# A-SHOJAEI/adverse-weather-semantic-segmentation-robustness-benchmark

Measured on AMD Instinct MI355X. Metric: images/sec (1024x2048, 5 weather conds, ensemble eval), higher is better.
Workload: dtype f32 (results float32; attention, gemm_1x1, winograd_3x3, segformer_head on 3xf16 split operands: 22-bit operands, f32 accumulate)

## Files before the change

adverse_weather_semantic_segmentation_robustness_benchmark_amd/_native.py:

```python
from __future__ import annotations

import ctypes as C
from pathlib import Path

import numpy as np
import torch

_PKG = Path(__file__).resolve().parent
LIB_PATH = _PKG / "libawseg_hip.so"

U8, I64 = 0, 1
COMBINE_WEIGHTED, COMBINE_MAXCONF, COMBINE_MEAN = 0, 1, 2
LOSS_CE, LOSS_FOCAL = 0, 1
ACT_NONE, ACT_RELU, ACT_GELU = 0, 1, 2
MAX_CLASSES = 32

c_i, c_i64, c_u64, c_f, c_d, c_p = C.c_int, C.c_int64, C.c_uint64, C.c_float, C.c_double, C.c_void_p

FOG_JOB = np.dtype([("image", "<i4"), ("_pad", "<i4"), ("beta", "<f8"), ("atmos", "<f8"), ("seed", "<u8")], align=True)
NIGHT_JOB = np.dtype([("image", "<i4"), ("_pad", "<i4"), ("brightness", "<f8"), ("intensity", "<f8"), ("seed", "<u8")], align=True)
PRIM_JOB = np.dtype([("image", "<i4"), ("prim_offset", "<i4"), ("prim_count", "<i4"), ("blur_ksize", "<i4"), ("intensity", "<f8")], align=True)
WEATHER_JOB = np.dtype([("kind", "<i4"), ("image", "<i4"), ("a", "<f8"), ("b", "<f8"), ("seed", "<u8"), ("prim_offset", "<i4"), ("prim_count", "<i4")], align=True)
WEATHER_CLEAN, WEATHER_FOG, WEATHER_RAIN, WEATHER_SNOW, WEATHER_NIGHT = 0, 1, 2, 3, 4
assert FOG_JOB.itemsize == 32 and NIGHT_JOB.itemsize == 32 and PRIM_JOB.itemsize == 24 and WEATHER_JOB.itemsize == 40

SIGNATURES = {
    "awseg_abi_version": (c_i, []),
    "awseg_header_hash": (C.c_uint64, []),
    "awseg_error_string": (C.c_char_p, [c_i]),
    "awseg_device_count": (c_i, []),
    "awseg_metrics_workspace": (c_i64, [c_i64, c_i, c_i64]),
    "awseg_confusion_accumulate": (c_i, [c_p, c_i, c_p, c_i, c_i64, c_i, c_i, c_i, c_p, c_p, c_p, c_p]),
    "awseg_argmax": (c_i, [c_p, c_i64, c_i, c_i64, c_p, c_i, c_p]),
    "awseg_combine_argmax_confusion": (c_i, [c_p, c_p, c_i64, c_i, c_i64, c_i, c_p, c_p, c_p, c_p, c_i, c_p, c_i, c_i,
                                            c_i, c_p, c_p, c_i, c_p, c_p, c_p]),
    "awseg_argmax_confusion": (c_i, [c_p, c_i64, c_i, c_i64, c_p, c_i, c_p, c_i, c_i, c_i, c_p, c_p, c_i, c_p, c_p, c_p]),
    "awseg_normalize": (c_i, [c_p, c_i64, c_i, c_i, c_p, c_i, c_p, c_p, c_p, c_p]),
    "awseg_synthetic_depth": (c_i, [c_i, c_i, c_p, c_i, c_p, c_p, c_p, c_p]),
    "awseg_conv3x3_winograd_nhwc": (c_i, [c_p, c_i, c_i, c_i, c_i, c_i, c_i, c_p, c_p, c_p, c_i, c_p, c_p, c_p, c_p]),
    "awseg_gemm_bias_act": (c_i, [c_p, c_p, c_p, c_p, c_i, c_p, c_i64, c_i, c_i, c_p, C.c_size_t, c_p]),
    "awseg_gemm_tune": (c_i, [c_p, c_p, c_p, c_i, c_i, c_p, c_i64, c_i, c_i, c_p, C.c_size_t, c_p]),
    "awseg_gemm_split_weights": (c_i, [c_p, c_i, c_i, c_p, c_p]),
    "awseg_gemm_split_weight_halfs": (c_i64, [c_i, c_i]),
    "awseg_gemm_split_bias_act": (c_i, [c_p, c_p, c_p, c_p, c_i, c_p, c_i64, c_i, c_i, c_p]),
    "awseg_gemm_bf16_weights": (c_i, [c_p, c_i, c_i, c_p, c_p]),
    "awseg_gemm_bf16_weight_halfs": (c_i64, [c_i, c_i]),
    "awseg_gemm_bf16_bias_act": (c_i, [c_p, c_p, c_p, c_p, c_i, c_p, c_i64, c_i, c_i, c_p]),
    "awseg_conv3x3_winograd_bf16_nhwc": (c_i, [c_p, c_i, c_i, c_i, c_i, c_i, c_i, c_p, c_p, c_p, c_i, c_p, c_p, c_p, c_p]),
    "awseg_attention_d32_bf16": (c_i, [c_p, c_p, c_p, c_p, c_i, c_i, c_i, c_i, c_f, c_p]),
    "awseg_attention_d32_split_workspace": (c_i64, [c_i, c_i, c_i]),
    "awseg_attention_d32_split_ws": (c_i, [c_p, c_p, c_p, c_i, c_p, c_i, c_i, c_i, c_i, c_f, c_p, c_p]),
    "awseg_attention_d32_packed_kv": (c_i, [c_p, c_p, c_p, c_i, c_i, c_i, c_i, c_f, c_i, c_p]),
    "awseg_dwconv3x3_upcat_nhwc": (c_i, [c_p, c_i, c_i, c_i, c_p, c_i, c_i64, c_i, c_i, c_p, c_p, c_p]),
    "awseg_winograd_split_weight_halfs": (c_i64, [c_i, c_i]),
    "awseg_conv3x3_winograd_split_nhwc": (c_i, [c_p, c_i, c_i, c_i, c_i, c_i, c_i, c_p, c_p, c_p, c_i, c_p, c_p, c_p, c_p]),
    "awseg_upconv_forms_floats": (c_i64, [c_i, c_i, c_i]),
    "awseg_upconv_forms": (c_i, [c_p, c_i, c_i, c_i, c_i, c_p, c_p, c_p]),
    "awseg_depth_head_fused": (c_i, [c_p, c_i, c_i, c_i, c_i, c_p, c_i, c_p, c_p, c_p, c_p, c_p]),
    "awseg_im2col_nhwc": (c_i, [c_p, c_i64, c_i, c_i, c_i, c_i, c_i, c_i, c_i, c_i, c_i, c_p, c_p]),
    "awseg_attention_d32": (c_i, [c_p, c_p, c_p, c_p, c_i, c_i, c_i, c_i, c_f, c_p]),
    "awseg_attention_d32_split": (c_i, [c_p, c_p, c_p, c_p, c_i, c_i, c_i, c_i, c_f, c_p]),
    "awseg_depth_upsample_combine": (c_i, [c_p, c_p, c_i, c_i, c_i, c_i, c_i, c_p, c_p, c_p, c_p]),
    "awseg_lut3_apply": (c_i, [c_p, c_i, c_i, c_i, c_p, c_i, c_p, c_p, c_p]),
    "awseg_local_contrast": (c_i, [c_p, c_i, c_i, c_i, c_p, c_p]),
    "awseg_depth_estimate_workspace": (C.c_size_t, [c_i]),
    "awseg_depth_estimate": (c_i, [c_p, c_i, c_i, c_i, c_p, c_p, c_p, c_p, c_p]),
    "awseg_fog_apply": (c_i, [c_p, c_i, c_i, c_p, c_i, c_p, c_p, c_p, c_p, c_p, c_p]),
    "awseg_fog_fused": (c_i, [c_p, c_i, c_i, c_p, c_i, c_p, c_p, c_p, c_p, c_p, c_p, c_p, c_p]),
    "awseg_night_apply": (c_i, [c_p, c_i, c_i, c_p, c_i, c_p, c_p, c_p, c_p, c_p, c_p, c_p]),
    "awseg_rain_apply": (c_i, [c_p, c_i, c_i, c_p, c_i, c_p, c_p, c_p, c_p, c_p, c_p, c_p]),
    "awseg_snow_apply": (c_i, [c_p, c_i, c_i, c_p, c_i, c_p, c_p, c_p, c_p, c_p, c_p, c_p]),
    "awseg_weather_batch": (c_i, [c_p, c_i, c_i, c_p, c_i, c_p, c_p, c_p, c_p, c_p, c_p, c_p, c_p, c_p, c_p]),
    "awseg_streak_workspace": (c_i64, [c_i, c_i, c_i]),
    "awseg_fog_density_field": (c_i, [c_p, c_i, c_i64, c_u64, c_p, c_p, c_p]),
    "awseg_loss_partials": (c_i64, [c_i64, c_i64]),
    "awseg_fog_ce_forward": (c_i, [c_p, c_p, c_i, c_p, c_i64, c_i, c_i64, c_i, c_f, c_p, c_p, c_p, c_p, c_p]),
    "awseg_fog_ce_backward": (c_i, [c_p, c_p, c_i, c_p, c_i64, c_i, c_i64, c_i, c_f, c_p, c_p, c_p]),
    "awseg_density_workspace": (c_i64, [c_i64, c_i64]),
    "awseg_fog_density_from_depth": (c_i, [c_p, c_i64, c_i, c_i, c_p, c_p, c_p]),
    "awseg_segformer_head_fused": (c_i, [c_p, c_i64, c_i, c_i, c_i, c_i, c_i, c_p, c_p, c_p, c_p, c_i, c_p, c_p]),
    "awseg_segformer_head_fused_split": (c_i, [c_p, c_i64, c_i, c_i, c_i, c_i, c_i, c_p, c_p, c_p, c_p, c_i, c_p, c_p]),
    "awseg_upconv3x3_bn_relu": (c_i, [c_p, c_i64, c_i, c_i, c_i, c_i, c_i, c_p, c_p, c_p, c_i, c_p]),
    "awseg_upconv3x3_linear": (c_i, [c_p, c_i64, c_i, c_i, c_i, c_i, c_i, c_p, c_p, c_i, c_p]),
    "awseg_upconv3x3_adjoint": (c_i, [c_p, c_i64, c_i, c_i, c_i, c_i, c_i, c_p, c_p]),
    "awseg_aspp_depthwise3": (c_i, [c_p, c_i64, c_i, c_i, c_i, c_p, c_i, c_i, c_i, c_p, c_p]),
    "awseg_aspp_depthwise3_mean": (c_i, [c_p, c_i64, c_i, c_i, c_i, c_p, c_i, c_i, c_i, c_p, c_p, c_p]),
# ... 148 lines not shown
```

adverse_weather_semantic_segmentation_robustness_benchmark_amd/csrc/build.py:

```python
from __future__ import annotations

import os
import shutil
import subprocess
import sys
from concurrent.futures import ThreadPoolExecutor
from pathlib import Path

CSRC = Path(__file__).resolve().parent
PKG = CSRC.parent
LIB = PKG / "libawseg_hip.so"
SOURCES = ["core.hip", "metrics.hip", "weather.hip", "loss.hip", "heads.hip", "backbone.hip", "depth.hip", "wino.hip", "gemm.hip", "attn.hip", "gemm_split.hip", "gemm_split3.hip", "wino_split.hip", "depthfuse.hip", "mixffn.hip", "dwtrain.hip", "bntrain.hip", "smallops.hip", "calib.hip", "consistency.hip", "deptheval.hip", "failure.hip"]
ARCH = "gfx950"
HEADER = PKG.parent / "include" / "awseg.h"


def header_hash() -> int:
    import hashlib
    return int(hashlib.sha256(HEADER.read_bytes()).hexdigest()[:15], 16)


EXTRA_FLAGS = {"attn.hip": ["-DAWSEG_ATTN_SPLIT_WAVES=" + os.environ.get("AWSEG_ATTN_SPLIT_WAVES", "2")], "wino.hip": ["-fno-slp-vectorize"], "wino_split.hip": ["-fno-slp-vectorize", "-DAWSEG_WS_ASM_PK"],
               "core.hip": ["-DAWSEG_HEADER_HASH=0x%xULL" % header_hash()]}


def hipcc() -> str:
    for cand in (os.environ.get("HIPCC"), "/opt/rocm/bin/hipcc", shutil.which("hipcc")):
        if cand and Path(cand).exists():
            return cand
    raise RuntimeError("hipcc not found (need ROCm's hipcc to build libawseg_hip.so)")


def _flags():
    return [f"--offload-arch={ARCH}", "-O3", "-std=c++17", "-fPIC", "-ffp-contract=off",
            "-fvisibility=hidden", "-Wall", "-Wno-unused-function", "-Wno-inline-asm"]


STAMP = PKG / "libawseg_hip.flags"


def _flag_stamp() -> str:
    return repr((_flags(), sorted(EXTRA_FLAGS.items()), SOURCES))


def needs_build() -> bool:
# ... 38 lines not shown
```

adverse_weather_semantic_segmentation_robustness_benchmark_amd/models/deeplab.py:

```python
from __future__ import annotations

import os

from typing import List

import torch
import torch.nn as nn
import torch.nn.functional as F

from .. import ops


class Conv2d(nn.Conv2d):

    linear_in_training = True
    keep_channels_last = os.environ.get("AWSEG_TRAIN_KEEP_CL", "1") != "0"
    matmul_nchw = os.environ.get("AWSEG_TRAIN_MATMUL_NCHW", "1") != "0"

    def forward(self, x: torch.Tensor) -> torch.Tensor:
        if (Conv2d.linear_in_training and x.is_cuda and torch.is_grad_enabled() and self.kernel_size == (1, 1) and self.groups == 1
                and self.padding == (0, 0) and x.dim() == 4 and x.shape[2] * x.shape[3] > 1):
            if self.stride != (1, 1):
                x = x[:, :, ::self.stride[0], ::self.stride[1]]
            b, c, h, w = x.shape
# ... 208 lines not shown
            dw, gmean = ops.aspp_depthwise3_mean(xl, wdw, aspp.rates)
        else:
            dw, gmean = ops.aspp_depthwise3(xl, wdw, aspp.rates), None
        dw = dw.view(3, B * h * w, Cin)
        if gmean is None:
            gmean = xl.mean(dim=(1, 2))
        pool = aspp.convs[4]
        pw_, pbn_ = pool[1].weight.view(Cout, Cin), pool[2]
        if xl.is_cuda and xl.dtype == torch.float32:
            def fold_pool():
                s_, b_ = _bn_fold(pbn_)
                return (pw_ * s_[:, None]).contiguous(), b_.contiguous()
            w1f, b1f = fused.cached(pbn_, "aspp_pool_fold", (pw_, pbn_.weight, pbn_.bias, pbn_.running_mean, pbn_.running_var), fold_pool)
            g2 = ops.aspp_pool_branch(gmean, w1f, b1f, parts[4], pb)
        else:
            g2 = branch(gmean, pw_, pbn_) @ parts[4].t() + pb
        acc = g2[:, None, :].expand(B, h * w, Cout).contiguous().view(B * h * w, Cout)
        ys = [branch(flat, aspp.convs[0][0].weight.view(Cout, Cin), aspp.convs[0][1])]
        for r in range(3):
            mod = aspp.convs[1 + r]
            ys.append(branch(dw[r], mod[0][1].weight.view(Cout, Cin), mod[1]))
        done = None
        if ops.ASPP_PIECES and ops.GEMM_SPLIT and ops.PRECISION != "bf16" and acc.is_cuda and Cout % 32 == 0:
            wcat = fused.cached(aspp.project[0], "proj_pieces", (parts[0], parts[1], parts[2], parts[3]),
                                lambda: ops.gemm_split_weights(torch.cat(parts[:4], dim=1).contiguous()))
            done = ops.gemm_split_pieces(ys, wcat, zero_bias, 1, residual=acc, out=acc)
        if done is None:
            for i, y in enumerate(ys):
                ops.gemm_bias_act(y, parts[i], zero_bias, 1 if i == 3 else 0, residual=acc, out=acc, w_split=psplit[i])
        out = acc
        return out.view(B, h, w, Cout).permute(0, 3, 1, 2)

    @torch.no_grad()
    def forward_fused(self, *features):
        from . import fused
        from .. import _native as N
        a = self.aspp_fused(features[-1])
        a = fused.separable_bn_relu(a, self.aspp[1], self.aspp[2])
        hi = fused.conv_bn_act(features[-4], self.block1[0], self.block1[1], N.ACT_RELU)
        dwc, pwc = self.block2[0][0], self.block2[0][1]
        d = ops.dwconv3x3_upcat(fused.nhwc_view(a), fused.nhwc_view(hi), fused.dw_taps(dwc))
        B, H4, W4, Cc = d.shape
        w, shift = fused.folded_conv_bn(pwc, self.block2[1])
        w2 = w.view(w.shape[0], Cc)
        y = ops.gemm_bias_act(d.view(B * H4 * W4, Cc), w2, shift, N.ACT_RELU, w_split=fused.split_weights(pwc, w2, B * H4 * W4))
        return y.view(B, H4, W4, -1).permute(0, 3, 1, 2)


class SegmentationHead(nn.Sequential):
    def __init__(self, in_ch, out_ch, kernel_size=1, upsampling=4):
        super().__init__(Conv2d(in_ch, out_ch, kernel_size, padding=kernel_size // 2),
                         nn.UpsamplingBilinear2d(scale_factor=upsampling) if upsampling > 1 else nn.Identity(),
                         nn.Identity())


class DeepLabV3Plus(nn.Module):

    def __init__(self, encoder_name="resnet50", classes=19, encoder_output_stride=16, decoder_channels=256,
                 decoder_atrous_rates=(12, 24, 36), upsampling=4):
        super().__init__()
        self.encoder = ResNetEncoder(encoder_name, encoder_output_stride)
        self.decoder = DeepLabV3PlusDecoder(self.encoder.out_channels, decoder_channels, decoder_atrous_rates,
                                            encoder_output_stride)
        self.segmentation_head = SegmentationHead(decoder_channels, classes, 1, upsampling)
        for m in list(self.decoder.modules()) + list(self.segmentation_head.modules()):
            if isinstance(m, nn.Conv2d):
                nn.init.kaiming_uniform_(m.weight, mode="fan_in", nonlinearity="relu")
                if m.bias is not None:
                    nn.init.constant_(m.bias, 0)
            elif isinstance(m, nn.BatchNorm2d):
                nn.init.constant_(m.weight, 1)
                nn.init.constant_(m.bias, 0)
        nn.init.xavier_uniform_(self.segmentation_head[0].weight)

    def forward(self, x):
        feats = self.encoder(x)
        return self.segmentation_head(self.decoder(*feats))

    @torch.no_grad()
    def forward_fused(self, x, return_features=False):
        from . import fused
        feats = fused.resnet_features(self.encoder, x)
        dec = self.decoder.forward_fused(*feats)
        head = self.segmentation_head[0]
        if head.kernel_size == (1, 1):
            dl = fused.nhwc_view(dec)
            Bq, H4, W4, Cd = dl.shape
            y2 = ops.gemm_bias_act(dl.reshape(Bq * H4 * W4, Cd), head.weight.view(head.out_channels, Cd), head.bias, 0,
                                   w_split=fused.split_weights(head, head.weight.view(head.out_channels, Cd), Bq * H4 * W4))
            low = y2.view(Bq, H4, W4, -1).permute(0, 3, 1, 2)
        else:
            low = head(dec).contiguous()
        up = self.segmentation_head[1]
        if isinstance(up, nn.UpsamplingBilinear2d) and low.is_cuda and low.dtype == torch.float32:
            f = int(up.scale_factor)
            out = ops.upsample_bilinear(low, (low.shape[2] * f, low.shape[3] * f), True)
        else:
            out = up(low)
        return (out, feats[-1]) if return_features else out
```

adverse_weather_semantic_segmentation_robustness_benchmark_amd/ops.py:

```python
from __future__ import annotations

import math
import os

import ctypes as C
from typing import Optional, Sequence

import numpy as np
import torch

from . import _native as N

IMAGENET_MEAN = np.array([0.485, 0.456, 0.406], dtype=np.float32)
IMAGENET_STD = np.array([0.229, 0.224, 0.225], dtype=np.float32)
NIGHT_GAINS = np.array([0.8, 0.85, 1.2], dtype=np.float32)
CONDITIONS = ("clean", "fog", "rain", "snow", "night")


def gaussian_taps(sigma: float = 2.0, truncate: float = 4.0) -> np.ndarray:
    radius = int(truncate * float(sigma) + 0.5)
    x = np.arange(-radius, radius + 1)
    phi = np.exp(-0.5 / (sigma * sigma) * x ** 2)
    return phi / phi.sum()

# ... 1058 lines not shown
    if k != kh * kw * c:
        raise N.AwsegError(f"conv_gemm_split: weights have K = {k}, the convolution needs {kh * kw * c}")
    if not _split_weights_intact(w_split, n, k):
        raise N.AwsegError("w_split lost its 16-byte trailer (weight exponent): pass the tensor gemm_split_weights returned, not a copy")
    ho = (h + 2 * pad - dilation * (kh - 1) - 1) // stride + 1
    wo = (w + 2 * pad - dilation * (kw - 1) - 1) // stride + 1
    out = torch.empty(b, ho, wo, n, dtype=torch.float32, device=x.device)
    N.call("awseg_conv_gemm_split_bias_act", N.ptr(x), b, h, w, c, kh, kw, stride, pad, dilation, N.ptr(w_split), N.ptr(bias),
           N.ptr(residual), act, N.ptr(out), n, N.stream())
    return out


def im2col_nhwc(x: torch.Tensor, kh: int, kw: int, stride: int, pad: int, dilation: int = 1, k_padded: Optional[int] = None):
    x = x.contiguous()
    b, h, w, c = x.shape
    k = kh * kw * c
    kp = k if k_padded is None else int(k_padded)
    ho = (h + 2 * pad - dilation * (kh - 1) - 1) // stride + 1
    wo = (w + 2 * pad - dilation * (kw - 1) - 1) // stride + 1
    cols = torch.empty(b * ho * wo, kp, dtype=torch.float32, device=x.device)
    N.call("awseg_im2col_nhwc", N.ptr(x), b, h, w, c, kh, kw, stride, pad, dilation, kp, N.ptr(cols), N.stream())
    return cols, ho, wo


def dwconv3x3_upcat(a: torch.Tensor, hi: torch.Tensor, w9: torch.Tensor) -> torch.Tensor:
    a, hi = a.contiguous(), hi.contiguous()
    b, h, w, ca = a.shape
    _, H, W, ch = hi.shape
    out = torch.empty(b, H, W, ca + ch, dtype=torch.float32, device=a.device)
    N.call("awseg_dwconv3x3_upcat_nhwc", N.ptr(a), h, w, ca, N.ptr(hi), ch, b, H, W, N.ptr(w9.contiguous()), N.ptr(out), N.stream())
    return out


ATTENTION_SPLIT = os.environ.get("AWSEG_ATTN_SPLIT", "1") != "0"


def attention_d32(q: torch.Tensor, k: torch.Tensor, v: torch.Tensor, heads: int, scale: float,
                  split: Optional[bool] = None) -> torch.Tensor:
    q, k, v = q.contiguous(), k.contiguous(), v.contiguous()
    b, nq, c = q.shape
    out = torch.empty_like(q)
    if split is None and PRECISION == "bf16":
        sym = "awseg_attention_d32_bf16"
    else:
        sym = "awseg_attention_d32_split" if (ATTENTION_SPLIT if split is None else split) else "awseg_attention_d32"
    if sym == "awseg_attention_d32_split" and _wants_kv_image(nq, k.shape[1]):
        _attention_split_ws(q, k, v, 0, out, b, heads, nq, k.shape[1], scale)
        return out
    N.call(sym, N.ptr(q), N.ptr(k), N.ptr(v), N.ptr(out), b, heads, nq, k.shape[1], float(scale), N.stream())
    return out


ATTN_KV_IMAGE = os.environ.get("AWSEG_ATTN_KV_IMAGE", "1") != "0"


def _wants_kv_image(nq: int, nkv: int) -> bool:
    return ATTN_KV_IMAGE and nq >= 8 * nkv


def _attention_split_ws(q, k, v, pitch, out, b, heads, nq, nkv, scale):
    nbytes = int(N.lib().awseg_attention_d32_split_workspace(b, heads, nkv))
    ws = N.workspace.get(q.device, nbytes, tag="attn%d" % torch.cuda.current_stream(q.device).cuda_stream)
    N.call("awseg_attention_d32_split_ws", N.ptr(q), N.ptr_strided(k), N.ptr_strided(v), int(pitch), N.ptr(out), b, heads, nq, nkv, float(scale),
           N.ptr(ws), N.stream())


# ... 153 lines not shown
```

include/awseg.h:

```cpp
#ifndef AWSEG_H
#define AWSEG_H

#include <stddef.h>
#include <stdint.h>

#ifdef __cplusplus
extern "C" {
#endif

typedef void* awseg_stream_t;

#define AWSEG_EINVAL   (-1)
#define AWSEG_ERANGE   (-2)
#define AWSEG_EALIGN   (-3)

#define AWSEG_U8   0
#define AWSEG_I64  1

#define AWSEG_COMBINE_WEIGHTED  0
#define AWSEG_COMBINE_MAXCONF   1
#define AWSEG_COMBINE_MEAN      2

#define AWSEG_LOSS_CE     0
#define AWSEG_LOSS_FOCAL  1
// ... 160 lines not shown
                            float* out, int channels_last, awseg_stream_t stream);

int awseg_aspp_depthwise3(const float* x, int64_t batch, int h, int w, int channels,
                          const float* wdw, int rate0, int rate1, int rate2,
                          float* out, awseg_stream_t stream);
int awseg_aspp_depthwise3_mean(const float* x, int64_t batch, int h, int w, int channels, const float* wdw,
                               int rate0, int rate1, int rate2, float* out, float* mean_out, awseg_stream_t stream);

#define AWSEG_ACT_NONE 0
#define AWSEG_ACT_RELU 1
#define AWSEG_ACT_GELU 2
int awseg_dwconv3x3_nhwc(const float* x, int64_t batch, int height, int width, int channels, int dilation,
                         const float* w9, const float* bias, int act, float* out, awseg_stream_t stream);

int awseg_conv3x3_winograd_nhwc(const float* x, int batch, int height, int width, int cin, int cout, int dilation,
                                const float* u, const float* shift, const float* residual, int act,
                                const float* w2, const float* b2, float* out, awseg_stream_t stream);

int awseg_gemm_bias_act(const float* x, const float* w, const float* bias, const float* residual, int act,
                        float* out, int64_t m, int n, int k, void* workspace, size_t workspace_bytes,
                        awseg_stream_t stream);

int awseg_gemm_tune(const float* x, const float* w, const float* bias, int has_residual, int act,
                    float* scratch_out, int64_t m, int n, int k, void* workspace, size_t workspace_bytes,
                    awseg_stream_t stream);

int64_t awseg_gemm_split_weight_halfs(int n, int k);
int awseg_gemm_split_weights(const float* w, int n, int k, uint16_t* w_split, awseg_stream_t stream);
int awseg_gemm_split_bias_act(const float* x, const uint16_t* w_split, const float* bias, const float* residual, int act,
                              float* out, int64_t m, int n, int k, awseg_stream_t stream);

int awseg_dwconv3x3_upcat_nhwc(const float* a, int a_height, int a_width, int a_channels, const float* hi, int hi_channels,
                               int64_t batch, int height, int width, const float* w9, float* out, awseg_stream_t stream);

int64_t awseg_winograd_split_weight_halfs(int cin, int cout);

int64_t awseg_upconv_forms_floats(int h, int w, int cmid);
int awseg_upconv_forms(const float* g9, int batch, int cmid, int h, int w, const float* shift, float* forms, awseg_stream_t stream);
int awseg_depth_head_fused(const float* forms, int batch, int h, int w, int cmid, const uint16_t* u_split, int u_is_bf16,
                           const float* shift2, const float* w2, const float* b2, float* out, awseg_stream_t stream);
int awseg_conv3x3_winograd_split_nhwc(const float* x, int batch, int height, int width, int cin, int cout, int dilation,
                                      const uint16_t* u_split, const float* shift, const float* residual, int act,
                                      const float* w2, const float* b2, float* out, awseg_stream_t stream);

int awseg_gemm_split_pieces_bias_act(const float* const* pieces, int n_pieces, int k_piece, const uint16_t* w_split, const float* bias,
                                     const float* residual, int act, float* out, int64_t m, int n, awseg_stream_t stream);

int awseg_gemm_split_dual_bias_act(const float* x, int k1, const float* x2, int k2, int64_t batch, int x2_height, int x2_width,
                                   int x2_stride, const uint16_t* w_split, const float* bias, const float* residual, int act,
                                   float* out, int64_t m, int n, awseg_stream_t stream);

int awseg_conv_gemm_split_bias_act(const float* x, int64_t batch, int height, int width, int channels,
                                   int kernel_h, int kernel_w, int stride, int pad, int dilation,
                                   const uint16_t* w_split, const float* bias, const float* residual, int act,
                                   float* out, int n, awseg_stream_t stream);

int awseg_conv_rows_gemm_split_bias_act(const float* x, int64_t batch, int height, int width_padded, int pixel_floats,
                                        int kernel_h, int stride, int pad_y, int out_width, const uint16_t* w_split,
                                        const float* bias, const float* residual, int act, float* out, int n,
                                        awseg_stream_t stream);

int64_t awseg_gemm_bf16_weight_halfs(int n, int k);
int awseg_gemm_bf16_weights(const float* w, int n, int k, uint16_t* w_bf16, awseg_stream_t stream);
int awseg_gemm_bf16_bias_act(const float* x, const uint16_t* w_bf16, const float* bias, const float* residual, int act,
                             float* out, int64_t m, int n, int k, awseg_stream_t stream);
int awseg_conv3x3_winograd_bf16_nhwc(const float* x, int batch, int height, int width, int cin, int cout, int dilation,
// ... 165 lines not shown
```

Baseline: 233.1.

## Fuse DeepLab decoder pointwise conv and segmentation head into one persistent kernel

```diff
diff --git a/adverse_weather_semantic_segmentation_robustness_benchmark_amd/_native.py b/adverse_weather_semantic_segmentation_robustness_benchmark_amd/_native.py
--- a/adverse_weather_semantic_segmentation_robustness_benchmark_amd/_native.py
+++ b/adverse_weather_semantic_segmentation_robustness_benchmark_amd/_native.py
@@ -52,6 +52,9 @@
     "awseg_attention_d32_split_ws": (c_i, [c_p, c_p, c_p, c_i, c_p, c_i, c_i, c_i, c_i, c_f, c_p, c_p]),
     "awseg_attention_d32_packed_kv": (c_i, [c_p, c_p, c_p, c_i, c_i, c_i, c_i, c_f, c_i, c_p]),
     "awseg_dwconv3x3_upcat_nhwc": (c_i, [c_p, c_i, c_i, c_i, c_p, c_i, c_i64, c_i, c_i, c_p, c_p, c_p]),
+    "awseg_deeplab_decoder_tail_weight_halfs": (c_i64, [c_i, c_i]),
+    "awseg_deeplab_decoder_tail_weights": (c_i, [c_p, c_i, c_i, c_p, c_p]),
+    "awseg_deeplab_decoder_tail": (c_i, [c_p, c_i64, c_i, c_p, c_p, c_i, c_p, c_p, c_i, c_p, c_p]),
     "awseg_winograd_split_weight_halfs": (c_i64, [c_i, c_i]),
     "awseg_conv3x3_winograd_split_nhwc": (c_i, [c_p, c_i, c_i, c_i, c_i, c_i, c_i, c_p, c_p, c_p, c_i, c_p, c_p, c_p, c_p]),
     "awseg_upconv_forms_floats": (c_i64, [c_i, c_i, c_i]),
diff --git a/adverse_weather_semantic_segmentation_robustness_benchmark_amd/csrc/build.py b/adverse_weather_semantic_segmentation_robustness_benchmark_amd/csrc/build.py
--- a/adverse_weather_semantic_segmentation_robustness_benchmark_amd/csrc/build.py
+++ b/adverse_weather_semantic_segmentation_robustness_benchmark_amd/csrc/build.py
@@ -10,7 +10,7 @@
 CSRC = Path(__file__).resolve().parent
 PKG = CSRC.parent
 LIB = PKG / "libawseg_hip.so"
-SOURCES = ["core.hip", "metrics.hip", "weather.hip", "loss.hip", "heads.hip", "backbone.hip", "depth.hip", "wino.hip", "gemm.hip", "attn.hip", "gemm_split.hip", "gemm_split3.hip", "wino_split.hip", "depthfuse.hip", "mixffn.hip", "dwtrain.hip", "bntrain.hip", "smallops.hip", "calib.hip", "consistency.hip", "deptheval.hip", "failure.hip"]
+SOURCES = ["core.hip", "metrics.hip", "weather.hip", "loss.hip", "heads.hip", "backbone.hip", "depth.hip", "wino.hip", "gemm.hip", "attn.hip", "gemm_split.hip", "gemm_split3.hip", "dectail.hip", "wino_split.hip", "depthfuse.hip", "mixffn.hip", "dwtrain.hip", "bntrain.hip", "smallops.hip", "calib.hip", "consistency.hip", "deptheval.hip", "failure.hip"]
 ARCH = "gfx950"
 HEADER = PKG.parent / "include" / "awseg.h"
 
diff --git a/adverse_weather_semantic_segmentation_robustness_benchmark_amd/csrc/dectail.hip b/adverse_weather_semantic_segmentation_robustness_benchmark_amd/csrc/dectail.hip
--- /dev/null
+++ b/adverse_weather_semantic_segmentation_robustness_benchmark_amd/csrc/dectail.hip
@@ -0,0 +1,419 @@
+#include "awseg_common.h"
+
+namespace {
+
+typedef float f32x16 __attribute__((ext_vector_type(16)));
+typedef float f32x4 __attribute__((ext_vector_type(4)));
+typedef _Float16 h8 __attribute__((ext_vector_type(8)));
+typedef unsigned u32x4 __attribute__((ext_vector_type(4)));
+
+constexpr int DTM = 256, DTK = 32, DTN = 256;
+constexpr int DT_STAGE = DTM * 128;
+constexpr int DT_LDS = 4 * DT_STAGE + 64 + DTN * 4;
+constexpr int DT_CP = 32;
+constexpr float kActScale0 = 16.0f;
+constexpr int kActExp0 = -4;
+constexpr float kSplitLimit = 2048.0f;
+constexpr float kSmallLimit = 0.0078125f;
+
+__device__ __forceinline__ float pow2fd(int e) { return __builtin_bit_cast(float, (unsigned)(127 + e) << 23); }
+
+__device__ __forceinline__ uint32_t lds_addr(const void* p)
+{
+    return (uint32_t)(uintptr_t)(__attribute__((address_space(3))) const void*)p;
+}
+__device__ __forceinline__ void dma16(__amdgpu_buffer_rsrc_t rsrc, uint32_t voff, uint32_t soff, uint32_t lds_base)
+{
+    asm volatile("s_mov_b32 m0, %3\n\ts_nop 0\n\tbuffer_load_dwordx4 %0, %1, %2 offen lds" : : "v"(voff), "s"(rsrc), "s"(soff), "s"(lds_base) : "m0", "memory");
+}
+__device__ __forceinline__ void split2(float a, float b, float s, unsigned& hi, unsigned& lo)
+{
+    asm("v_fma_mixlo_f16 %0, %2, %4, 0\n\t"
+        "v_fma_mixhi_f16 %0, %3, %4, 0\n\t"
+        "v_fma_mixlo_f16 %1, %2, %4, -%0 op_sel_hi:[0,0,1]\n\t"
+        "v_fma_mixhi_f16 %1, %3, %4, -%0 op_sel:[0,0,1] op_sel_hi:[0,0,1]\n\t"
+        "s_nop 1"
+        : "=&v"(hi), "=&v"(lo) : "v"(a), "v"(b), "s"(s));
+}
+
+#ifdef AWSEG_DT_STAMP
+__device__ unsigned long long g_dt_stamp[2][8];
+#define DT_T(v) const unsigned long long v = __builtin_readcyclecounter()
+#else
+#define DT_T(v)
+#endif
+
+struct dt_args {
+    const float* x;
+    const uint16_t* w3;
+    const unsigned* tr1;
+    const float* bias1;
+    const uint16_t* w2i;
+    const float* bias2;
+    float* out;
+    int64_t M; int K, classes, ntm;
+    float floor1, floor2;
+    int stagger;
+};
+
+__global__ __launch_bounds__(512, 2)
+void decoder_tail_kernel(dt_args a)
+{
+    extern __shared__ __attribute__((aligned(16))) unsigned char smem[];
+    unsigned* sMax = reinterpret_cast<unsigned*>(smem + 4 * DT_STAGE);
+    float* sBias = reinterpret_cast<float*>(smem + 4 * DT_STAGE + 64);
+    const int tid = threadIdx.x, lane = tid & 63, wave = tid >> 6;
+    const int hk = lane >> 5, li = lane & 31;
+    const int K = a.K, nkt = (K + DTK - 1) / DTK;
+    const int ktail = K % DTK;
+
+    const int rl = lane >> 3, sl = lane & 7;
+    uint32_t a_voff[4], a_voff_last[4], b_voff[4];
+    const uint32_t lds0 = __builtin_amdgcn_readfirstlane(lds_addr(smem));
+    const uint32_t wave_u = __builtin_amdgcn_readfirstlane(wave);
+    __amdgpu_buffer_rsrc_t x_rsrc;
+    const __amdgpu_buffer_rsrc_t w_rsrc = __builtin_amdgcn_make_buffer_rsrc((void*)a.w3, 0, DTN * nkt * 128, 0x00020000);
+    const __amdgpu_buffer_rsrc_t w2_rsrc = __builtin_amdgcn_make_buffer_rsrc((void*)a.w2i, 0, (DTN / DTK) * DT_CP * 128, 0x00020000);
+#pragma unroll
+    for (int j = 0; j < 4; ++j) {
+        const int row = 8 * (4 * wave + j) + rl;
+        const int c = sl ^ ((row >> 1) & 7);
+        a_voff[j] = (uint32_t)(row * K * 4 + c * 16);
+        a_voff_last[j] = (ktail == 0 || c * 4 < ktail) ? a_voff[j] : 0x80000000u;
+        b_voff[j] = (uint32_t)(row * 128 + c * 16);
+    }
+    auto point = [&](int64_t m0) {
+        const int64_t xbytes = (a.M - m0) * (int64_t)K * 4;
+        x_rsrc = __builtin_amdgcn_make_buffer_rsrc((void*)(a.x + m0 * K), 0, (int)(xbytes > 0x7fffffff ? 0x7fffffff : xbytes), 0x00020000);
+    };
+    auto issue = [&](int kt, int stage) {
+        const uint32_t la = lds0 + (uint32_t)(stage * DT_STAGE) + wave_u * 4096u;
+        const uint32_t lb = la + (uint32_t)(2 * DT_STAGE);
+#pragma unroll
+        for (int j = 0; j < 4; ++j) dma16(x_rsrc, kt == nkt - 1 ? a_voff_last[j] : a_voff[j], (uint32_t)(kt * 128), la + (uint32_t)(j * 1024));
+#pragma unroll
+        for (int j = 0; j < 4; ++j) dma16(w_rsrc, b_voff[j], (uint32_t)(kt * DTN * 128), lb + (uint32_t)(j * 1024));
+    };
+
+    const int sw = (li >> 1) & 7;
+    int fa[2][2], fb[2][2];
+#pragma unroll
+    for (int ks = 0; ks < 2; ++ks) {
+#pragma unroll
+        for (int e = 0; e < 2; ++e) fa[ks][e] = (wave * 32 + li) * 128 + (((4 * ks + 2 * hk + e) ^ sw) * 16);
+        fb[ks][0] = 2 * DT_STAGE + li * 128 + (((2 * ks + hk) ^ sw) * 16);
+        fb[ks][1] = 2 * DT_STAGE + li * 128 + (((4 + 2 * ks + hk) ^ sw) * 16);
+    }
+    const unsigned* tr2 = reinterpret_cast<const unsigned*>(a.w2i + (DTN / DTK) * DT_CP * 64);
+
+    int tile = blockIdx.x;
+    if (tile >= a.ntm) return;
+    if (tid < 4) sMax[tid] = 0u;
+    if (tid < DTN) sBias[tid] = a.bias1[tid];
+    int par = 0;
+    const int we1 = (int)a.tr1[1], we2 = (int)tr2[1];
+    float amax = 0.f, sx = kActScale0;
+    int xe = kActExp0;
+    bool scaled = false;
+    int g = 0;
+    int64_t m0 = (int64_t)tile * DTM;
+#ifdef AWSEG_DT_STAMP
+    unsigned long long dts[7] = {0, 0, 0, 0, 0, 0, 0};
+#endif
+    point(m0);
+    issue(0, 0);
+
+    while (true) {
+        const int ntile = tile + (int)gridDim.x;
+        const bool has_next = ntile < a.ntm;
+
+        f32x16 acc[8];
+#pragma unroll
+        for (int j = 0; j < 8; ++j)
+#pragma unroll
+            for (int r = 0; r < 16; ++r) acc[j][r] = 0.f;
+        amax = 0.f;
+
+        for (int t = 0; t < nkt; ++t, ++g) {
+            const int st = g & 1;
+            DT_T(s0);
+            asm volatile("s_waitcnt vmcnt(0)" ::: "memory");
+            __builtin_amdgcn_s_barrier();
+            DT_T(s1);
+            const bool issue_late = a.stagger && wave_u >= 4;
+            if (t + 1 < nkt && !issue_late) issue(t + 1, st ^ 1);
+            if (t == 0 && tid == 0) { sMax[par ^ 1] = 0u; sMax[2 + (par ^ 1)] = 0u; }
+            const unsigned char* sa = smem + st * DT_STAGE;
+#pragma unroll
+            for (int ks = 0; ks < 2; ++ks) {
+                if (ks == 1 && t + 1 < nkt && issue_late) issue(t + 1, st ^ 1);
+                const f32x4 p = *reinterpret_cast<const f32x4*>(sa + fa[ks][0]);
+                const f32x4 q = *reinterpret_cast<const f32x4*>(sa + fa[ks][1]);
+                h8 Bh[8], Bl[8];
+#pragma unroll
+                for (int j = 0; j < 8; ++j) {
+                    Bh[j] = *reinterpret_cast<const h8*>(sa + fb[ks][0] + j * 4096);
+                    Bl[j] = *reinterpret_cast<const h8*>(sa + fb[ks][1] + j * 4096);
+                }
+                amax = __builtin_fmaxf(__builtin_fmaxf(amax, __builtin_fabsf(p[0])), __builtin_fabsf(p[1]));
+                amax = __builtin_fmaxf(__builtin_fmaxf(amax, __builtin_fabsf(p[2])), __builtin_fabsf(p[3]));
+                amax = __builtin_fmaxf(__builtin_fmaxf(amax, __builtin_fabsf(q[0])), __builtin_fabsf(q[1]));
+                amax = __builtin_fmaxf(__builtin_fmaxf(amax, __builtin_fabsf(q[2])), __builtin_fabsf(q[3]));
+                u32x4 H, L; unsigned h, l;
+                split2(p[0], p[1], sx, h, l); H[0] = h; L[0] = l;
+                split2(p[2], p[3], sx, h, l); H[1] = h; L[1] = l;
+                split2(q[0], q[1], sx, h, l); H[2] = h; L[2] = l;
+                split2(q[2], q[3], sx, h, l); H[3] = h; L[3] = l;
+                const h8 Ah = __builtin_bit_cast(h8, H), Al = __builtin_bit_cast(h8, L);
+#pragma unroll
+                for (int j = 0; j < 8; ++j) {
+                    acc[j] = __builtin_amdgcn_mfma_f32_32x32x16_f16(Bh[j], Ah, acc[j], 0, 0, 0);
+                    acc[j] = __builtin_amdgcn_mfma_f32_32x32x16_f16(Bl[j], Ah, acc[j], 0, 0, 0);
+                    acc[j] = __builtin_amdgcn_mfma_f32_32x32x16_f16(Bh[j], Al, acc[j], 0, 0, 0);
+                }
+            }
+#ifdef AWSEG_DT_STAMP
+            { DT_T(s2); dts[0] += s1 - s0; dts[1] += s2 - s1; }
+#endif
+        }
+        DT_T(e0);
+
+        if (!scaled) {
+            const bool not_small = __ballot(amax >= kSmallLimit) != 0ull;
+            if (amax >= kSplitLimit || !not_small) atomicMax(&sMax[par], __builtin_bit_cast(unsigned, amax));
+            if (not_small && (tid & 63) == 0) sMax[2 + par] = 1u;
+        }
+        asm volatile("s_waitcnt lgkmcnt(0)" ::: "memory");
+        __builtin_amdgcn_s_barrier();
+        const unsigned mx = sMax[par];
+        const bool small = sMax[2 + par] == 0u;
+        par ^= 1;
+        constexpr unsigned kBig = __builtin_bit_cast(unsigned, kSplitLimit), kSmall = __builtin_bit_cast(unsigned, kSmallLimit);
+        if (!scaled && (mx >= kBig || (small && mx >= 0x00800000u && mx < kSmall))) {
+            const int ex = (int)(mx >> 23) & 0xff;
+            if (ex != 0xff) {
+                xe = ex - 127 - 13;
+                xe = xe < -127 ? -127 : xe;
+                sx = pow2fd(-xe);
+                scaled = true;
+                issue(0, g & 1);
+                continue;
+            }
+        }
+        const int64_t em0 = m0;
+        DT_T(e1);
+        if (has_next) { point((int64_t)ntile * DTM); issue(0, g & 1); }
+        const int wst = (g & 1) ^ 1;
+        {
+            const uint32_t lw = lds0 + (uint32_t)(wst * DT_STAGE) + wave_u * 4096u;
+#pragma unroll
+            for (int j = 0; j < 4; ++j) dma16(w2_rsrc, b_voff[j], 0u, lw + (uint32_t)(j * 1024));
+        }
+
+        float y[8][16];
+        {
+            const int oe = we1 + xe;
+            const int oe1 = oe / 2, oe2 = oe - oe1;
+            const float os1 = pow2fd(oe1 < -126 ? -126 : (oe1 > 127 ? 127 : oe1)), os2 = pow2fd(oe2 < -126 ? -126 : (oe2 > 127 ? 127 : oe2));
+            const f32x4* b1 = reinterpret_cast<const f32x4*>(sBias) + hk;
+#pragma unroll
+            for (int j = 0; j < 8; ++j) {
+                f32x4 bv[4];
+#pragma unroll
+                for (int g4 = 0; g4 < 4; ++g4) bv[g4] = b1[j * 8 + 2 * g4];
+#pragma unroll
+                for (int g4 = 0; g4 < 4; ++g4)
+#pragma unroll
+                    for (int e = 0; e < 4; ++e) {
+                        float vv = acc[j][4 * g4 + e] * os1 * os2;
+                        vv = vv + bv[g4][e];
+                        y[j][4 * g4 + e] = __builtin_fmaxf(vv, a.floor1);
+                    }
+            }
+        }
+        float sy = kActScale0; int ye = kActExp0;
+        {
+            float ymax = 0.f;
+#pragma unroll
+            for (int j = 0; j < 8; ++j)
+#pragma unroll
+                for (int r = 0; r < 16; r += 2) ymax = __builtin_fmaxf(__builtin_fmaxf(ymax, __builtin_fabsf(y[j][r])), __builtin_fabsf(y[j][r + 1]));
+            const bool y_not_small = __ballot(ymax >= kSmallLimit) != 0ull;
+            const bool y_big = __ballot(ymax >= kSplitLimit) != 0ull;
+            if (y_big || !y_not_small) {
+#pragma unroll
+                for (int o = 32; o > 0; o >>= 1) ymax = __builtin_fmaxf(ymax, __shfl_xor(ymax, o, 64));
+                const unsigned my = (unsigned)__builtin_amdgcn_readfirstlane((int)__builtin_bit_cast(unsigned, ymax));
+                if (my >= kBig || (my >= 0x00800000u && my < kSmall)) {
+                    const int ex = (int)(my >> 23) & 0xff;
+                    if (ex != 0xff) {
+                        ye = ex - 127 - 13;
+                        ye = ye < -127 ? -127 : ye;
+                        sy = pow2fd(-ye);
+                    }
+                }
+            }
+        }
+        f32x16 acc2;
+#pragma unroll
+        for (int r = 0; r < 16; ++r) acc2[r] = 0.f;
+        DT_T(e2);
+        asm volatile("s_waitcnt vmcnt(0)" ::: "memory");
+        __builtin_amdgcn_s_barrier();
+        DT_T(e3);
+        const int wo = wst * DT_STAGE - 2 * DT_STAGE;
+#pragma unroll
+        for (int t = 0; t < 8; ++t) {
+#pragma unroll
+            for (int ks = 0; ks < 2; ++ks) {
+                const h8 Wh = *reinterpret_cast<const h8*>(smem + (wo + fb[ks][0] + t * 4096));
+                const h8 Wl = *reinterpret_cast<const h8*>(smem + (wo + fb[ks][1] + t * 4096));
+                float p[4], q[4];
+#pragma unroll
+                for (int e = 0; e < 4; ++e) {
+                    const auto r2 = __builtin_amdgcn_permlane32_swap(__builtin_bit_cast(unsigned, y[t][8 * ks + e]),
+                                                                     __builtin_bit_cast(unsigned, y[t][8 * ks + 4 + e]), false, false);
+                    p[e] = __builtin_bit_cast(float, (unsigned)r2[0]);
+                    q[e] = __builtin_bit_cast(float, (unsigned)r2[1]);
+                }
+                u32x4 H, L; unsigned h, l;
+                split2(p[0], p[1], sy, h, l); H[0] = h; L[0] = l;
+                split2(p[2], p[3], sy, h, l); H[1] = h; L[1] = l;
+                split2(q[0], q[1], sy, h, l); H[2] = h; L[2] = l;
+                split2(q[2], q[3], sy, h, l); H[3] = h; L[3] = l;
+                const h8 Yh = __builtin_bit_cast(h8, H), Yl = __builtin_bit_cast(h8, L);
+                acc2 = __builtin_amdgcn_mfma_f32_32x32x16_f16(Yh, Wh, acc2, 0, 0, 0);
+                acc2 = __builtin_amdgcn_mfma_f32_32x32x16_f16(Yh, Wl, acc2, 0, 0, 0);
+                acc2 = __builtin_amdgcn_mfma_f32_32x32x16_f16(Yl, Wh, acc2, 0, 0, 0);
+            }
+        }
+        {
+            const int oe = we2 + ye;
+            const int oe1 = oe / 2, oe2 = oe - oe1;
+            const float os1 = pow2fd(oe1 < -126 ? -126 : (oe1 > 127 ? 127 : oe1)), os2 = pow2fd(oe2 < -126 ? -126 : (oe2 > 127 ? 127 : oe2));
+            const bool col_ok = li < a.classes;
+            const float bv = (a.bias2 && col_ok) ? a.bias2[li] : 0.f;
+            const int64_t row0 = em0 + wave * 32 + 4 * hk;
+#pragma unroll
+            for (int r = 0; r < 16; ++r) {
+                const int64_t row = row0 + (r & 3) + 8 * (r >> 2);
+                float vv = acc2[r] * os1 * os2;
+                vv = vv + bv;
+                vv = __builtin_fmaxf(vv, a.floor2);
+                if (col_ok && row < a.M) a.out[row * a.classes + li] = vv;
+            }
+        }
+#ifdef AWSEG_DT_STAMP
+        { asm volatile("s_waitcnt vmcnt(0)" ::: "memory"); DT_T(e4); dts[2] += e1 - e0; dts[3] += e2 - e1; dts[4] += e3 - e2; dts[5] += e4 - e3; dts[6] += 1; }
+#endif
+        if (!has_next) break;
+        tile = ntile; m0 = (int64_t)ntile * DTM;
+        scaled = false; sx = kActScale0; xe = kActExp0;
+    }
+#ifdef AWSEG_DT_STAMP
+    if (blockIdx.x == 0 && (tid == 0 || tid == 256))
+        for (int i = 0; i < 7; ++i) g_dt_stamp[tid >> 8][i] += dts[i];
+#endif
+}
+
+__device__ __forceinline__ int norm_exponent_d(unsigned maxbits)
+{
+    const int ex = (int)(maxbits >> 23) & 0xff;
+    if (ex == 0 || ex == 0xff) return 0;
+    return ex - 127 - 13;
+}
+
+__global__ __launch_bounds__(256)
+void decoder_tail_head_weights_kernel(const float* __restrict__ w, int classes, int k_dim, uint16_t* __restrict__ out)
+{
+    __shared__ unsigned s_max;
+    if (threadIdx.x == 0) s_max = 0u;
+    __syncthreads();
+    float m = 0.f;
+    for (int i = threadIdx.x; i < classes * k_dim; i += 256) m = fmaxf(m, fabsf(w[i]));
+    if (m > 0.f) atomicMax(&s_max, __builtin_bit_cast(unsigned, m));
+    __syncthreads();
+    const unsigned mb = s_max;
+    const int e = norm_exponent_d(mb);
+    const int e1 = e / 2, e2 = e - e1;
+    const float s1 = pow2fd(-e1), s2 = pow2fd(-e2);
+    const int kb = k_dim / DTK;
+    if (threadIdx.x == 0) {
+        unsigned* trailer = reinterpret_cast<unsigned*>(out + kb * DT_CP * 64);
+        trailer[0] = mb; trailer[1] = (unsigned)e; trailer[2] = 0u; trailer[3] = 0u;
+    }
+    for (int i = threadIdx.x; i < DT_CP * k_dim; i += 256) {
+        const int n = i / k_dim, k = i - n * k_dim;
+        const float x = n < classes ? w[n * k_dim + k] * s1 * s2 : 0.f;
+        const _Float16 h = (_Float16)x;
+        const _Float16 l = (_Float16)(x - (float)h);
+        uint16_t* d = out + ((k >> 5) * DT_CP + n) * 64 + (k & 31);
+        d[0] = __builtin_bit_cast(uint16_t, h);
+        d[32] = __builtin_bit_cast(uint16_t, l);
+    }
+}
+
+}
+
+AWSEG_API int64_t awseg_deeplab_decoder_tail_weight_halfs(int classes, int hidden)
+{
+    if (classes < 1 || classes > DT_CP || hidden != DTN) return -1;
+    return (int64_t)(hidden / DTK) * DT_CP * 64 + 8;
+}
+
+AWSEG_API int awseg_deeplab_decoder_tail_weights(const float* w2, int classes, int hidden, uint16_t* w2_image, awseg_stream_t stream)
+{
+    if (!w2 || !w2_image) return AWSEG_EINVAL;
+    if (classes < 1 || classes > DT_CP || hidden != DTN) return AWSEG_ERANGE;
+    if ((uintptr_t)w2_image & 15) return AWSEG_EALIGN;
+    hipLaunchKernelGGL(decoder_tail_head_weights_kernel, dim3(1), dim3(256), 0, awseg_s(stream), w2, classes, hidden, w2_image);
+    AWSEG_LAUNCH_CHECK();
+    return 0;
+}
+
+AWSEG_API int awseg_deeplab_decoder_tail(const float* d, int64_t m, int k, const uint16_t* w1_split, const float* bias1, int hidden,
+                                         const uint16_t* w2_image, const float* bias2, int classes, float* out, awseg_stream_t stream)
+{
+    if (m == 0) return 0;
+    if (!d || !w1_split || !bias1 || !w2_image || !out || m < 0) return AWSEG_EINVAL;
+    if (hidden != DTN || classes < 1 || classes > DT_CP || k < DTK || k % 8) return AWSEG_ERANGE;
+    if ((int64_t)DTM * (k + DTK) * 4 > 0x7fffffff || (m + DTM - 1) / DTM > 0x7fffffff) return AWSEG_ERANGE;
+    if (((uintptr_t)d | (uintptr_t)w1_split | (uintptr_t)bias1 | (uintptr_t)w2_image) & 15) return AWSEG_EALIGN;
+    if (((uintptr_t)out | (uintptr_t)bias2) & 3) return AWSEG_EALIGN;
+    dt_args a;
+    const int64_t ne = (int64_t)hidden * k;
+    a.x = d; a.tr1 = reinterpret_cast<const unsigned*>(w1_split + 2 * ne); a.w3 = w1_split + 2 * ne + 8;
+    a.bias1 = bias1; a.w2i = w2_image; a.bias2 = bias2; a.out = out;
+    a.M = m; a.K = k; a.classes = classes; a.ntm = (int)((m + DTM - 1) / DTM);
+    a.floor1 = 0.f; a.floor2 = -__builtin_inff();
+    static int stagger = -1;
+    if (stagger < 0) { const char* e = getenv("AWSEG_G3_STAGGER"); stagger = e ? atoi(e) : 1; }
+    a.stagger = stagger;
+    static int cus = 0;
+    if (cus == 0) {
+        int dev = 0, n_cu = 0;
+        if (hipGetDevice(&dev) != hipSuccess || hipDeviceGetAttribute(&n_cu, hipDeviceAttributeMultiprocessorCount, dev) != hipSuccess || n_cu < 1) n_cu = 256;
+        cus = n_cu;
+    }
+    int blocks = cus / 8 * 8;
+    if (blocks < 8) blocks = 8;
+    if (blocks > a.ntm) blocks = a.ntm;
+    static bool attr = false;
+    if (!attr) {
+        hipError_t e = hipFuncSetAttribute(reinterpret_cast<const void*>(decoder_tail_kernel), hipFuncAttributeMaxDynamicSharedMemorySize, DT_LDS);
+        if (e != hipSuccess) return (int)e;
+        attr = true;
+    }
+    hipLaunchKernelGGL(decoder_tail_kernel, dim3((unsigned)blocks), dim3(512), DT_LDS, awseg_s(stream), a);
+    AWSEG_LAUNCH_CHECK();
+    return 0;
+}
+
+#ifdef AWSEG_DT_STAMP
+AWSEG_API int awseg_debug_dt_stamps(unsigned long long* out16, int reset)
+{
+    hipError_t e = hipMemcpyFromSymbol(out16, HIP_SYMBOL(g_dt_stamp), sizeof(unsigned long long) * 16);
+    if (e == hipSuccess && reset) { unsigned long long z[16] = {}; e = hipMemcpyToSymbol(HIP_SYMBOL(g_dt_stamp), z, sizeof z); }
+    return (int)e;
+}
+#endif
diff --git a/adverse_weather_semantic_segmentation_robustness_benchmark_amd/models/deeplab.py b/adverse_weather_semantic_segmentation_robustness_benchmark_amd/models/deeplab.py
--- a/adverse_weather_semantic_segmentation_robustness_benchmark_amd/models/deeplab.py
+++ b/adverse_weather_semantic_segmentation_robustness_benchmark_amd/models/deeplab.py
@@ -264,12 +264,39 @@
         return out.view(B, h, w, Cout).permute(0, 3, 1, 2)
 
     @torch.no_grad()
-    def forward_fused(self, *features):
+    def fused_branches(self, *features):
         from . import fused
         from .. import _native as N
         a = self.aspp_fused(features[-1])
         a = fused.separable_bn_relu(a, self.aspp[1], self.aspp[2])
         hi = fused.conv_bn_act(features[-4], self.block1[0], self.block1[1], N.ACT_RELU)
+        return a, hi
+
+    @torch.no_grad()
+    def forward_fused_logits(self, head: nn.Conv2d, *features):
+        from . import fused
+        dwc, pwc = self.block2[0][0], self.block2[0][1]
+        if not (head.kernel_size == (1, 1) and head.in_channels == pwc.out_channels and head.weight.is_cuda and head.weight.dtype == torch.float32
+                and ops.decoder_tail_fits(dwc.in_channels - self.block1[0].out_channels, self.block1[0].out_channels, pwc.out_channels, head.out_channels)):
+            return None
+        lo_f, hi_f = features[-1], features[-4]
+        if hi_f.shape[2] != 4 * lo_f.shape[2] or hi_f.shape[3] != 4 * lo_f.shape[3]:
+            return None
+        a, hi = self.fused_branches(*features)
+        w, shift = fused.folded_conv_bn(pwc, self.block2[1])
+        w1 = w.view(w.shape[0], dwc.in_channels)
+        w1_split = fused.cached(pwc, "wsplit", (w1,), lambda: ops.gemm_split_weights(w1))
+        classes, Cd = head.out_channels, head.in_channels
+        w2_image = fused.cached(head, "tail_w2", (head.weight,), lambda: ops.deeplab_decoder_tail_weights(head.weight.view(classes, Cd)))
+        return ops.deeplab_decoder_tail(fused.nhwc_view(a), fused.nhwc_view(hi), fused.dw_taps(dwc), w1_split, shift, w2_image, head.bias, classes)
+
+    @torch.no_grad()
+    def forward_fused(self, *features):
+        return self._block2_fused(*self.fused_branches(*features))
+
+    def _block2_fused(self, a, hi):
+        from . import fused
+        from .. import _native as N
         dwc, pwc = self.block2[0][0], self.block2[0][1]
         d = ops.dwconv3x3_upcat(fused.nhwc_view(a), fused.nhwc_view(hi), fused.dw_taps(dwc))
         B, H4, W4, Cc = d.shape
@@ -313,9 +340,12 @@
     def forward_fused(self, x, return_features=False):
         from . import fused
         feats = fused.resnet_features(self.encoder, x)
-        dec = self.decoder.forward_fused(*feats)
         head = self.segmentation_head[0]
-        if head.kernel_size == (1, 1):
+        tail = self.decoder.forward_fused_logits(head, *feats) if x.is_cuda else None
+        dec = None if tail is not None else self.decoder.forward_fused(*feats)
+        if tail is not None:
+            low = tail.permute(0, 3, 1, 2)
+        elif head.kernel_size == (1, 1):
             dl = fused.nhwc_view(dec)
             Bq, H4, W4, Cd = dl.shape
             y2 = ops.gemm_bias_act(dl.reshape(Bq * H4 * W4, Cd), head.weight.view(head.out_channels, Cd), head.bias, 0,
diff --git a/adverse_weather_semantic_segmentation_robustness_benchmark_amd/ops.py b/adverse_weather_semantic_segmentation_robustness_benchmark_amd/ops.py
--- a/adverse_weather_semantic_segmentation_robustness_benchmark_amd/ops.py
+++ b/adverse_weather_semantic_segmentation_robustness_benchmark_amd/ops.py
@@ -1114,6 +1114,48 @@
     return out
 
 
+DECODER_TAIL = os.environ.get("AWSEG_DECODER_TAIL", "1") != "0"
+DECODER_TAIL_HIDDEN, DECODER_TAIL_MAX_CLASSES = 256, 32
+
+
+def decoder_tail_fits(ca: int, ch: int, hidden: int, classes: int) -> bool:
+    return (DECODER_TAIL and GEMM_SPLIT and PRECISION != "bf16" and hidden == DECODER_TAIL_HIDDEN
+            and 1 <= classes <= DECODER_TAIL_MAX_CLASSES and ca % 32 == 0 and ch % 8 == 0)
+
+
+def deeplab_decoder_tail_weights(w2: torch.Tensor) -> torch.Tensor:
+    w2 = w2.contiguous()
+    classes, hidden = w2.shape
+    halfs = int(N.lib().awseg_deeplab_decoder_tail_weight_halfs(classes, hidden))
+    if halfs < 0:
+        raise N.AwsegError(f"deeplab_decoder_tail_weights: [{classes}, {hidden}] head weights are not served")
+    img = torch.empty(halfs, dtype=torch.int16, device=w2.device)
+    N.call("awseg_deeplab_decoder_tail_weights", N.ptr(w2), classes, hidden, N.ptr(img), N.stream())
+    return img
+
+
+def deeplab_decoder_tail_rows(d: torch.Tensor, w1_split: torch.Tensor, bias1: torch.Tensor, w2_image: torch.Tensor,
+                              bias2: Optional[torch.Tensor], classes: int) -> torch.Tensor:
+    d = d.contiguous()
+    m, k = d.shape
+    hidden = w1_split.shape[1]
+    if w1_split.shape[2] != k:
+        raise N.AwsegError(f"deeplab_decoder_tail: weights have K = {w1_split.shape[2]}, the depthwise map {k} channels")
+    if not _split_weights_intact(w1_split, hidden, k):
+        raise N.AwsegError("w1_split lost its 16-byte trailer (weight exponent): pass the tensor gemm_split_weights returned, not a copy")
+    out = torch.empty(m, classes, dtype=torch.float32, device=d.device)
+    N.call("awseg_deeplab_decoder_tail", N.ptr(d), m, k, N.ptr(w1_split), N.ptr(bias1.contiguous()), hidden, N.ptr(w2_image),
+           N.ptr(None if bias2 is None else bias2.contiguous()), classes, N.ptr(out), N.stream())
+    return out
+
+
+def deeplab_decoder_tail(a: torch.Tensor, hi: torch.Tensor, w9: torch.Tensor, w1_split: torch.Tensor, bias1: torch.Tensor,
+                         w2_image: torch.Tensor, bias2: Optional[torch.Tensor], classes: int) -> torch.Tensor:
+    d = dwconv3x3_upcat(a, hi, w9)
+    b, H, W, k = d.shape
+    return deeplab_decoder_tail_rows(d.view(b * H * W, k), w1_split, bias1, w2_image, bias2, classes).view(b, H, W, classes)
+
+
 ATTENTION_SPLIT = os.environ.get("AWSEG_ATTN_SPLIT", "1") != "0"
 
 
diff --git a/include/awseg.h b/include/awseg.h
--- a/include/awseg.h
+++ b/include/awseg.h
@@ -216,6 +216,11 @@
 
 int awseg_dwconv3x3_upcat_nhwc(const float* a, int a_height, int a_width, int a_channels, const float* hi, int hi_channels,
                                int64_t batch, int height, int width, const float* w9, float* out, awseg_stream_t stream);
+
+int64_t awseg_deeplab_decoder_tail_weight_halfs(int classes, int hidden);
+int awseg_deeplab_decoder_tail_weights(const float* w2, int classes, int hidden, uint16_t* w2_image, awseg_stream_t stream);
+int awseg_deeplab_decoder_tail(const float* d, int64_t m, int k, const uint16_t* w1_split, const float* bias1, int hidden,
+                               const uint16_t* w2_image, const float* bias2, int classes, float* out, awseg_stream_t stream);
 
 int64_t awseg_winograd_split_weight_halfs(int cin, int cout);
 
```

Result: no change. 234.4 (median of 6 runs) (+0.6%).
